# ExaScience/elprep

Measured on AMD Instinct MI355X. Metric: Mreads/s through sort+markdup+BQSR, 150bp PE, higher is better.
Workload: dtype u8/int32/int64 (integer path; float64 finalize on host)

## Files before the change

elprep_amd/csrc/bqsr.hip:

```cpp
#include <utility>

#include "bqsr_common.hpp"

namespace elp {

__global__ __launch_bounds__(256) void k_pack_reference(const uint8_t *__restrict__ ascii, int64_t len, uint8_t *__restrict__ packed, int64_t packed_bytes) {
  const int64_t i = (int64_t)blockIdx.x * blockDim.x + threadIdx.x;
  if (i >= packed_bytes) return;
  uint32_t out = 0;
  for (int h = 0; h < 2; h++) {
    const int64_t j = 2 * i + h;
    uint32_t code = 8;
    if (j < len) {
      switch (ascii[j]) {
        case 'a': case 'A': case '*': code = 0; break;
        case 'c': case 'C': code = 1; break;
        case 'g': case 'G': code = 2; break;
        case 't': case 'T': code = 3; break;
        default: code = 8;
      }
    }
    out |= code << (4 * h);
  }
  packed[i] = (uint8_t)out;
// ... 175 lines not shown
  ELP_TRY(fetch_err(c, e));
  if (e[0]) return bqsr_error(c, e[0]);
  const int64_t *hp = static_cast<const int64_t *>(c->h_pinned);
  memcpy(qual_tbl, hp, nq * 8);
  memcpy(cycle_tbl, hp + nq, nc * 8);
  memcpy(ctx_tbl, hp + nq + nc, nx * 8);
  return 0;
}

static int gather_impl(elp_ctx *c, int max_cycle, int64_t *qual_tbl, int64_t *cycle_tbl, int64_t *ctx_tbl) {
  for (int r = 0; r < c->n_ref; r++)
    if (!c->h_ref_seq[r]) return set_error(c, ELP_ERR_ARG, "elp_bqsr_gather: no reference sequence set for refid %d", r);
  for (int r = 0; r < c->n_ref; r++)
    if (!c->h_sites[r]) ELP_TRY(elp_bqsr_set_known_sites(c, r, nullptr, 0));
  ELP_TRY(sync_bqsr_ptrs(c));
  ELP_TRY(ensure_adapted(c, false));
  ELP_TRY(ensure_flat_index(c));
  ELP_TRY(ensure_qual_present(c));
  if (c->n_cov > 255) return set_error(c, ELP_ERR_UNSUPPORTED, "more than 255 read-group covariates");
  if (c->cigar_ops + 4 * c->n >= 0x7FFFFFFFull) return set_error(c, ELP_ERR_UNSUPPORTED, "CIGAR pool exceeds 2^31 operations per context");
  const int ncyc_g = 2 * max_cycle + 1;
  const size_t nq = (size_t)c->n_cov * ELP_NQUAL * 2, nc = nq * ncyc_g, nx = nq * ELP_NCTX;
  c->tables_n = 0;
  ELP_TRY(ensure(c, c->dev_tables, nq + nc + nx + elp_ctx::TABLES_TAIL));
  unsigned long long *tb = c->dev_tables.p;
  hipStream_t st = c->stream;
  ELP_HIP(c, hipMemsetAsync(tb, 0, (nq + nc + nx) * sizeof(unsigned long long), st));
  const uint64_t n = c->n;
  if (n && c->qual_bytes) {
    const GatherScratch S(n);
    PrologueBufs b;
    ELP_TRY(scratch(c, 1, 2 * (c->cigar_ops + 4 * n) + 64, &b.cs_pool));
    ELP_TRY(scratch(c, 2, n + 4, &b.desc));
    ELP_TRY(scratch(c, 0, 4 * n + 8, &b.plain_rec));
    const size_t skip_words = (size_t)((c->qual_bytes + 31) / 32 + 8);
    ELP_TRY(scratch(c, 3, skip_words, &b.skipbits));
    ELP_TRY(ensure_uniform_len(c));
    ELP_TRY(scratch(c, 5, S.words, &b.block));
    ELP_HIP(c, hipMemsetAsync(b.block, 0, 16, st));
    const GatherShape g{c->n_cov, (int)std::max<uint32_t>(c->max_l_seq, 1), max_cycle, c->uniform_len, c->tune.count_kernel, c->tune.count3_rlog,
                        COUNT3_STATIC_LDS, COUNT_STATIC_LDS, COUNT_STATIC_LDS_1024};
    uint32_t ncs = 1;
    while ((int)ncs < c->n_cov) ncs <<= 1;
    int mode = c3_mode(g, (int)quality_slots(c).size());
    if (S.too_many()) return set_error(c, ELP_ERR_UNSUPPORTED, "BQSR: more than ~1.4 G records per context");
    RecOut ro;
    ELP_TRY(rec_buffers(c, S, b.block, mode, ncs, &ro));
    if (!ro.recs) ELP_HIP(c, hipMemsetAsync(b.skipbits, 0, skip_words * 4, st));
    ELP_TRY(prologue_launch(c, b, S, ro));
    if (g.lmax > MAX_DESC_READ) return set_error(c, ELP_ERR_UNSUPPORTED, "BQSR: read longer than %d bases", MAX_DESC_READ);
    for (int attempt = 0;; attempt++) {
      const std::vector<int> quals = quality_slots(c);
      const CountPlan p = count_general_plan(g, (int)quals.size());
      if (!p.fits) return set_error(c, ELP_ERR_UNSUPPORTED, "BQSR: one covariate's private table rows do not fit in LDS (max read length=%d)", g.lmax);
      const int mode2 = ro.recs ? c3_mode(g, (int)quals.size()) : mode;
      if (mode2 != mode) {
        mode = mode2;
        ELP_TRY(rec_buffers(c, S, b.block, mode, ncs, &ro));
        ELP_HIP(c, hipMemsetAsync(b.skipbits, 0, skip_words * 4, st));
        ELP_HIP(c, hipMemsetAsync(b.block, 0, 16, st));
        ELP_TRY(prologue_launch(c, b, S, ro));
      }
      if (ro.recs) ELP_TRY(count_one_length(c, g, S, b, ro, quals, tb + nq, tb + nq + nc));
      else ELP_TRY(count_general(c, g, p, b, quals, tb + nq, tb + nq + nc));
      uint32_t e[4];
      ELP_TRY(fetch_err(c, e));
      if ((e[0] & ~128u) != 0) return bqsr_error(c, e[0] & ~128u);
// ... 160 lines not shown
```

elprep_amd/csrc/bqsr_common.hpp:

```cpp
#pragma once
#include "bqsr_dev.hpp"
#include "bqsr_plan.hpp"
#include "flat.hpp"

namespace elp {

constexpr int MAX_DESC_READ = 65535;


constexpr int32_t BQ_NOREF = INT32_MIN;
enum : uint8_t { BQ_ELIGIBLE = 1, BQ_REVERSED = 2, BQ_LAST = 4, BQ_CIG_SCRATCH = 8, BQ_COMPLEX = 16 };
struct __attribute__((aligned(16))) BqDesc {
  int32_t D0, D1, D2;
  int32_t refid;
  uint16_t b1, b2;
  uint16_t a;
  uint16_t len;
  uint16_t left;
  uint16_t right;
  uint8_t cov;
  uint8_t fl;
  uint16_t pad;
};
static_assert(sizeof(BqDesc) == 32, "BqDesc is staged as two 16-byte words");
// ... 231 lines not shown
  int rsw, rlog;
  unsigned long long *cycle_tbl, *ctx_tbl;
  uint32_t *err;
};
int count3_launch(elp_ctx *c, const Count3Args &A, const QMap &qm, size_t dyn);

struct CountArgs {
  uint64_t n, qual_bytes;
  const uint64_t *qual_off, *seq_off;
  const uint8_t *qual, *seq4;
  const BqDesc *desc;
  const uint32_t *cigar, *cig_scratch;
  const uint8_t *skipbits;
  uint8_t *const *ref_seq;
  const int64_t *ref_seq_len;
  int n_ref, n_cov, n_q, lmax, rs, max_cycle;
  unsigned long long *cycle_tbl, *ctx_tbl;
  uint32_t *err;
  const uint32_t *tile_first;
  int cov0;
};

int count_general_launch(elp_ctx *c, const CountArgs &A, const QMap &qm, const CountPlan &p, size_t dyn);
int qual_from_cycle_launch(elp_ctx *c, int ncyc_g, const unsigned long long *cycle_tbl, unsigned long long *qual_tbl);
int c3_segments_launch(elp_ctx *c, const GatherScratch &S, uint32_t *block, uint32_t nseg, uint32_t ncs);
int c3_other_sort_launch(elp_ctx *c, const uint4 *other, const uint32_t *n_other, uint32_t *cw, uint4 *sorted);

struct PrologueBufs {
  BqDesc *desc;
  uint32_t *skipbits;
  uint32_t *block;
  uint32_t *cs_pool;
  uint4 *plain_rec;
};
int prologue_launch(elp_ctx *c, const PrologueBufs &b, const GatherScratch &S, const RecOut &ro);

extern const size_t COUNT3_STATIC_LDS;
extern const size_t COUNT_STATIC_LDS, COUNT_STATIC_LDS_1024;
extern const size_t APPLY3_STATIC_LDS;

int bqsr_error(elp_ctx *c, uint32_t e);

int apply3_launch(elp_ctx *c, int max_cycle, const uint8_t *d_lut, const uint8_t *d_cov_present, const uint16_t *t1, const uint8_t *t2, const uint32_t *n_dict_dev,
                  int n_qi, int lmax, size_t dyn, bool split );

}
```

elprep_amd/csrc/bqsr_plan.hpp:

```cpp
#pragma once
#include <algorithm>
#include <cstddef>
#include <cstdint>

namespace elp {

constexpr size_t LDS_CU = 160 * 1024;

constexpr int CT_CYC = 32, CT_XROWS = 3, CT_PAD = 64;
constexpr int C3_XROWS = 3, C3_PAD = 64;
constexpr int C3_NSEG = 64;
constexpr int C3_MAXSEG = 256;
constexpr int C3_CSTRIDE = 64;
constexpr int PF_TILES = 16;
constexpr int CO_MAXCOV = 256;
constexpr int A3_ROW = 20;

inline int count3_plan(int n_cov, int n_q, int lmax, size_t static_lds, int *rsw_out, int *rlog_out, size_t *dyn_out, int force_rlog = -1) {
  const int ncw = ((17 * 2 * lmax) >> 4) + 2;
  const size_t rows = (size_t)n_cov * (size_t)(n_q + C3_XROWS);
  for (int rlog = 5; rlog >= 1; rlog--) {
    if (force_rlog >= 0 && force_rlog != rlog) continue;
    const int rsw = ((16 << rlog) + 16 + ncw + 31) & ~31;
    const size_t dyn = (rows * (size_t)rsw + C3_PAD) * 4;
    if (dyn + static_lds <= LDS_CU && rows * (size_t)rsw * 4 < (1u << 22)) {
      *rsw_out = rsw; *rlog_out = rlog; *dyn_out = dyn;
      return 0;
    }
  }
  return 1;
}

inline int apply3_bytes(int n_cov, int n_qi, int lmax, size_t static_lds, size_t *dyn_out) {
  const size_t n1 = (size_t)n_cov * (size_t)(6 + n_qi + 1) * (size_t)(2 * lmax + 1);
  const size_t dyn = ((n1 + 15) & ~(size_t)15) + (size_t)256 * A3_ROW + 16;
  *dyn_out = dyn;
  return dyn + static_lds <= LDS_CU ? 0 : 1;
}

struct GatherShape {
  int n_cov, lmax, max_cycle;
  uint32_t uniform_len;
  int count_kernel, count3_rlog;
  size_t lds_count3, lds_count, lds_count1024;
};

inline int c3_mode(const GatherShape &g, int nq) {
// ... 43 lines not shown
  p.passes = split(p.rs, &p.ncp, &p.qcap);
  if (p.passes != 1) {
    const int rs_mg = count_row_words(g.lmax, true);
    int ncp_mg = 0, qcap_mg = 0;
    const long passes_mg = split(rs_mg, &ncp_mg, &qcap_mg);
    if (passes_mg && (!p.passes || passes_mg < p.passes)) { p.mg = true; p.rs = rs_mg; p.ncp = ncp_mg; p.qcap = qcap_mg; p.passes = passes_mg; }
  }
  p.fits = p.qcap >= 1;
  return p;
}

struct GatherScratch {
  uint64_t n;
  size_t queue, plist, rec_cnt, cw, seg_cap, seg_base;
  size_t words;
  unsigned pf_grid;
  uint64_t cap_s1;
  explicit GatherScratch(uint64_t n_records) : n(n_records) {
    queue = 4;
    plist = (size_t)n + 20;
    rec_cnt = (size_t)((2 * n + 48 + 63) & ~(uint64_t)63);
    cw = rec_cnt + (size_t)(C3_MAXSEG + 1) * C3_CSTRIDE;
    seg_cap = cw + 3 * CO_MAXCOV + 1;
    seg_base = seg_cap + C3_MAXSEG;
    words = 2 * (size_t)n + 128 + (size_t)(C3_MAXSEG + 1) * C3_CSTRIDE + 4 * CO_MAXCOV + 2 * C3_MAXSEG + 32;
    pf_grid = (unsigned)((n + 256 * PF_TILES - 1) / (256 * PF_TILES));
    cap_s1 = ((uint64_t)pf_grid * 4 + C3_NSEG - 1) / C3_NSEG * (uint64_t)(PF_TILES * 64);
  }
  uint64_t other_at(int mode) const { return mode == 2 ? n : (uint64_t)C3_NSEG * cap_s1; }
  size_t rec_slots(int mode) const { return (size_t)other_at(mode) + (mode == 2 ? 2 : 1) * (size_t)n + 64; }
  bool too_many() const { return (uint64_t)C3_NSEG * cap_s1 + 2 * n >= 0xFFFFFFF0ull; }
};

}
```

elprep_amd/csrc/bqsr_prologue.hip:

```cpp
#include "bqsr_common.hpp"

namespace elp {

struct BqCols {
  uint64_t n;
  const int32_t *refid, *pos, *next_refid, *pnext, *tlen;
  const uint16_t *flag, *rgid;
  const uint8_t *mapq, *has_sr;
  const uint32_t *l_seq;
  const uint64_t *cigar_off, *seq_off, *qual_off;
  const uint32_t *cigar;
  const uint8_t *seq4;
  const uint8_t *qual;
  const int32_t *ref_len;
  const uint16_t *rg_cov;
  int32_t n_ref;
  uint8_t *const *ref_seq;
  const int64_t *ref_seq_len;
  int32_t *const *sites;
  const int64_t *n_sites;
  uint32_t *const *site_idx;
  const uint64_t *qbounds;
};

__device__ inline bool recalibrate_aln(const BqCols &m, uint64_t i) {
  if (m.has_sr[i]) return false;
  const uint8_t mq = m.mapq[i];
  if (!(mq > 0 && mq < 255)) return false;
  const uint16_t f = m.flag[i];
  if (f & (F_SECONDARY | F_DUPLICATE | F_QCFAILED)) return false;
  const int32_t r = m.refid[i], p = m.pos[i];
  if ((f & F_UNMAPPED) || r < 0 || p == 0) return false;
  if (!(p > 0)) return false;
  const uint32_t ls = m.l_seq[i];
  if (ls == 0) return false;
  if ((uint64_t)ls != m.qual_off[i + 1] - m.qual_off[i]) return false;
  if (m.rgid[i] == ELP_NIL16) return false;
  if (!(r < m.n_ref && p <= m.ref_len[r])) return false;
  int32_t rl = 0, refl = 0;
  for (uint64_t k = m.cigar_off[i]; k < m.cigar_off[i + 1]; k++) {
    const uint32_t c = m.cigar[k];
    if (c_op(c) == OP_N) return false;
    if (op_consumes_read(c_op(c))) rl += c_len(c);
    if (op_consumes_ref(c_op(c))) refl += c_len(c);
  }
  return refl >= 0 && (int32_t)ls == rl;
}

__device__ inline bool build_pieces(const uint32_t *cig, int ncig, int32_t pos, BqDesc &d) {
  int64_t val[3];
  bool noref[3];
  int start[3];
  int np = 0;
  int c = 0;
  int64_t delta = (int64_t)pos - 1;
// ... 23 lines not shown
    if (val[k] <= (int64_t)INT32_MIN + 70000 || val[k] >= (int64_t)INT32_MAX - 70000) return false;
    D[k] = (int32_t)val[k];
  }
  d.D0 = D[0]; d.D1 = D[1]; d.D2 = D[2];
  d.b1 = np > 1 ? (uint16_t)start[1] : (uint16_t)0xFFFF;
  d.b2 = np > 2 ? (uint16_t)start[2] : (uint16_t)0xFFFF;
  return true;
}

__device__ __forceinline__ void set_skip_bits(uint32_t *skipbits, uint64_t bit0, int fs, int fe) {
  for (int k = fs; k <= fe;) {
    const uint64_t b = bit0 + (uint64_t)k;
    const int in_word = (int)(b & 31);
    int cnt = 32 - in_word;
    if (cnt > fe - k + 1) cnt = fe - k + 1;
    const uint32_t mask = (cnt == 32 ? 0xFFFFFFFFu : ((1u << cnt) - 1u)) << in_word;
    atomicOr(&skipbits[b >> 5], mask);
    k += cnt;
  }
}

__device__ __forceinline__ void clear_skip_bits(uint32_t *skipbits, uint64_t bit0, uint32_t nbits) {
  for (uint32_t k = 0; k < nbits;) {
    const uint64_t b = bit0 + (uint64_t)k;
    const uint32_t in_word = (uint32_t)(b & 31);
    uint32_t cnt = 32 - in_word;
    if (cnt > nbits - k) cnt = nbits - k;
    const uint32_t mask = (cnt == 32 ? 0xFFFFFFFFu : ((1u << cnt) - 1u)) << in_word;
    atomicAnd(&skipbits[b >> 5], ~mask);
    k += cnt;
  }
}

struct PfCols {
  uint8_t has_sr, mq;
  uint16_t f, rg;
  int32_t r, p, pnext, tlen, nrefid;
  uint32_t ls;
  uint64_t q0, q1, c0, c1, qb;
};
__device__ __forceinline__ PfCols pf_load_cols(const BqCols &m, uint64_t i) {
  PfCols c;
  c.has_sr = m.has_sr[i]; c.mq = m.mapq[i]; c.f = m.flag[i]; c.rg = m.rgid[i];
  c.r = m.refid[i]; c.p = m.pos[i]; c.pnext = m.pnext[i]; c.tlen = m.tlen[i]; c.nrefid = m.next_refid[i];
  c.ls = m.l_seq[i];
  c.q0 = m.qual_off[i]; c.q1 = m.qual_off[i + 1]; c.c0 = m.cigar_off[i]; c.c1 = m.cigar_off[i + 1];
  c.qb = m.qbounds[i];
  return c;
}
struct PfLds {
  int32_t ref_len[REF_LDS];
  const int32_t *sites[REF_LDS];
  int64_t nsites[REF_LDS];
  const uint32_t *sidx[REF_LDS];
};
__device__ __forceinline__ void pf_lds_fill(PfLds &L, const BqCols &m, int nt) {
  if (m.n_ref <= REF_LDS)
    for (int r = threadIdx.x; r < m.n_ref; r += nt) { L.ref_len[r] = m.ref_len[r]; L.sites[r] = m.sites[r]; L.nsites[r] = m.n_sites[r]; L.sidx[r] = m.site_idx[r]; }
}

template <bool PLAIN_PASS>
__device__ __forceinline__ void pf_record(const BqCols &m, const uint64_t i, const PfCols &cur, const PfLds &L, const bool ref_lds, BqDesc *__restrict__ desc,
                                          uint32_t *skipbits, uint32_t *err, const bool recs , uint32_t *my_cig_w, bool &defer, bool &to_plain,
                                          BqRec &rc_out, int &rc_class, uint4 *__restrict__ plain_rec ,
                                          const uint32_t *pre_ops ) {
    const uint8_t has_sr = cur.has_sr, mq = cur.mq;
    const uint16_t f = cur.f, rg = cur.rg;
    const int32_t r = cur.r, p = cur.p, pnext = cur.pnext, tlen = cur.tlen, nrefid = cur.nrefid;
    const uint32_t ls = cur.ls;
    const uint64_t q0 = cur.q0, q1 = cur.q1, c0 = cur.c0, c1 = cur.c1;
    const uint64_t qb = cur.qb;
    BqDesc d;
    d.D0 = d.D1 = d.D2 = BQ_NOREF; d.refid = 0; d.b1 = d.b2 = 0xFFFF; d.a = 0; d.len = 0; d.left = 0; d.right = 0; d.cov = 0; d.fl = 0; d.pad = 0;
    const uint8_t *rec_rp = nullptr;
    int64_t rec_rlen = 0;
    bool used_col = false, rec_skipped_walk = false;
    bool ok = !has_sr && mq > 0 && mq < 255 && !(f & (F_SECONDARY | F_DUPLICATE | F_QCFAILED)) && !(f & F_UNMAPPED) && r >= 0 && p > 0 && ls != 0 &&
              (uint64_t)ls == q1 - q0 && rg != ELP_NIL16 && r < m.n_ref;
    if (ok) {
      const uint64_t nop = c1 - c0;
      if (recs) { rec_rp = m.ref_seq[r]; rec_rlen = m.ref_seq_len[r]; }
      uint32_t opv[5];
#pragma unroll
      for (int k = 0; k < 5; k++) opv[k] = PLAIN_PASS ? pre_ops[k] : ((uint64_t)k < nop ? m.cigar[c0 + k] : 0u);
      const int32_t rl = ref_lds ? L.ref_len[r] : m.ref_len[r];
      const uint16_t cov_rg = m.rg_cov[rg];
      const int32_t *sv = ref_lds ? L.sites[r] : m.sites[r];
      const int64_t ns = ref_lds ? L.nsites[r] : m.n_sites[r];
      auto bucket_entry = [&]() __attribute__((always_inline)) -> int64_t {
        const int64_t nbuck = ((int64_t)rl >> 6) + 1;
        int64_t bk = (int64_t)(p < rl ? p : rl) >> 6;
        bk = bk >= nbuck ? nbuck - 1 : bk;
        return (int64_t)(ref_lds ? L.sidx[r] : m.site_idx[r])[bk];
      };
      int64_t s_first = 0;
      if (!recs && ns > 0) s_first = bucket_entry();
      ok = p <= rl;
      bool simple = nop >= 1 && nop <= 5;
      uint32_t aoff = 0, mlen = 0, trail = 0;
      {
        uint32_t k = 0;
        if (simple && c_op(opv[0]) == OP_H) k = 1;
        auto at = [&](uint32_t j) { return j == 0 ? opv[0] : (j == 1 ? opv[1] : (j == 2 ? opv[2] : (j == 3 ? opv[3] : opv[4]))); };
        if (simple && k < nop && c_op(at(k)) == OP_S) { aoff = (uint32_t)c_len(at(k)); k++; }
        if (simple && k < nop && (c_op(at(k)) == OP_M || c_op(at(k)) == OP_EQ || c_op(at(k)) == OP_X)) { mlen = (uint32_t)c_len(at(k)); k++; }
        else simple = false;
        if (simple && k < nop && c_op(at(k)) == OP_S) { trail = (uint32_t)c_len(at(k)); k++; }
        if (simple && k < nop && c_op(at(k)) == OP_H) k++;
        simple = simple && k == nop && mlen != 0;
      }
      bool plain = false;
      uint32_t plain_read = 0, plain_ref = 0;
      if (!simple && nop >= 2 && nop <= 5) {
        plain = true;
#pragma unroll
        for (int k = 0; k < 5; k++) {
          if ((uint64_t)k < nop) {
            const uint32_t o = c_op(opv[k]), ln = (uint32_t)c_len(opv[k]);
            if (o == OP_M || o == OP_EQ || o == OP_X) { plain_read += ln; plain_ref += ln; }
            else if (o == OP_I) plain_read += ln;
            else if (o == OP_D) plain_ref += ln;
            else plain = false;
          }
        }
      }
      if (!PLAIN_PASS) {
        if (ok && plain && ls <= (uint32_t)MAX_DESC_READ) {
          uint4 *pr = plain_rec + 4 * i;
          pr[0] = make_uint4(opv[0], opv[1], opv[2], opv[3]);
          pr[1] = make_uint4(opv[4], (uint32_t)f | ((uint32_t)rg << 16), (uint32_t)r, (uint32_t)p);
          pr[2] = make_uint4(ls | ((uint32_t)nop << 16) | (nrefid < 0 ? 1u << 19 : 0u), (uint32_t)c0, (uint32_t)q0, (uint32_t)(q0 >> 32));
          pr[3] = make_uint4((uint32_t)qb, (uint32_t)(qb >> 32), (uint32_t)pnext, (uint32_t)tlen);
          to_plain = true;
          return;
        }
        plain = false;
      } else if (plain) {
#pragma unroll
        for (int k = 0; k < 5; k++) my_cig_w[k] = opv[k];
      }
      const uint32_t *my_cig = my_cig_w;
      if (ok && !((simple || plain) && ls <= (uint32_t)MAX_DESC_READ)) { defer = true; ok = false; }
      if (ok) ok = (plain ? plain_read : aoff + mlen + trail) == ls;
      if (ok) {
        const int len = plain ? (int)ls : (int)mlen;
        const int32_t end = p + (plain ? (int)plain_ref : len) - 1;
        const bool rev = f & F_REVERSED;
        bool clip = false;
        if (tlen != 0 && (f & F_MULTIPLE) && !((f & F_NEXT_UNMAPPED) || nrefid < 0 || pnext == 0) && rev != (bool)(f & F_NEXT_REVERSED)) {
          const bool well = rev ? end > pnext : p <= pnext + tlen;
          if (well) {
            const int boundary = rev ? (int)pnext - 1 : (int)p + (tlen < 0 ? -(int)tlen : (int)tlen);
            clip = boundary >= (int)p && boundary <= (int)end;
          }
        }
        const uint32_t hi1 = (uint32_t)qb;
        int left = len, right = len - 1;
        if (!clip && hi1) {
          const int f0 = (int)(qb >> 32) - (int)aoff, l0 = (int)hi1 - 1 - (int)aoff;
          if (f0 < len && l0 >= 0) {
            if (f0 >= 0) left = f0;
            else if (m.qual[q0 + aoff] > 2) left = 0;
            else clip = true;
            if (l0 < len) right = l0;
            else if (m.qual[q0 + aoff + (uint32_t)len - 1] > 2) right = len - 1;
            else clip = true;
// ... 45 lines not shown
            d.b1 = (uint16_t)nop;
            d.D2 = p - 1;
          }
          d.left = (uint16_t)left; d.right = (uint16_t)(right < 0 ? 0xFFFF : right);
          d.cov = (uint8_t)cov_rg;
          d.fl = BQ_ELIGIBLE | (rev ? BQ_REVERSED : 0) | ((f & F_LAST) ? BQ_LAST : 0) | complex_fl;
        }
      }
    }
    if (!defer) {
      if (recs) {
        BqRec rc;
        rc.ref_lo = rc.ref_hi = rc.win = rc.ctxw = 0; rc.t0 = 0; rc.fl = rc.bpk = rc.dpk = 0;
        if (d.fl & BQ_ELIGIBLE) {
          Pieces4 P;
          if (d.fl & BQ_COMPLEX) pieces4(my_cig_w, (int)(c1 - c0), p, P);
          else if (d.b1 != 0xFFFFu) pieces4(my_cig_w, (int)(c1 - c0), p, P);
          else { P.v0 = (int64_t)d.D0; P.v1 = P.v2 = P.v3 = 0; P.s1 = P.s2 = P.s3 = 0; P.noref = d.D0 == BQ_NOREF ? 1u : 0u; P.np = 1; }
          rc = make_rec((int)d.a, (int)d.len, (int)d.left, d.right == 0xFFFFu ? -1 : (int)d.right, d.cov, (d.fl & BQ_REVERSED) != 0, (d.fl & BQ_LAST) != 0, P,
                        P.np < 0, rec_rp, rec_rlen, (int64_t)ls);
          if (used_col) rc.fl |= RC_SKIPCOL;
          else if ((rc.fl & RC_GENERAL) && rec_skipped_walk) atomicOr(&err[0], 1024u);
        }
        if (rc.fl & RC_GENERAL) desc[i] = d;
        rc_class = rec_class(rc);
        rec_pack_idx(rc, (uint32_t)i);
        rc_out = rc;
      } else {
        desc[i] = d;
      }
    }
}

__global__ __launch_bounds__(256) void k_bqsr_prologue_fast(BqCols m, BqDesc *__restrict__ desc, uint32_t *skipbits, uint32_t *__restrict__ queue,
                                                            uint32_t *queue_n, uint32_t *err, RecOut ro, uint32_t *__restrict__ plist, uint4 *__restrict__ plain_rec) {
  __shared__ uint32_t lq[PF_TILES * 256];
  __shared__ uint32_t lcount, gbase, pcount, pbase;
  __shared__ uint32_t seg_n[C3_MAXSEG], seg_at[C3_MAXSEG];
  __shared__ PfLds L;
  const bool ref_lds = m.n_ref <= REF_LDS;
  pf_lds_fill(L, m, 256);
  if (threadIdx.x == 0) { lcount = 0; pcount = 0; }
  seg_n[threadIdx.x] = 0;
  __syncthreads();
  const uint64_t i_first = (uint64_t)blockIdx.x * PF_TILES * 256 + threadIdx.x;
  PfCols nxt = {};
  if (i_first < m.n) nxt = pf_load_cols(m, i_first);
#pragma unroll 1
  for (int tile = 0; tile < PF_TILES; tile++) {
    const uint64_t i = i_first + (uint64_t)tile * 256;
    bool defer = false, to_plain = false;
    const PfCols cur = nxt;
    if (tile + 1 < PF_TILES && i + 256 < m.n) nxt = pf_load_cols(m, i + 256);
    BqRec rc;
    int rcl = 0;
    if (i < m.n) pf_record<false>(m, i, cur, L, ref_lds, desc, skipbits, err, ro.recs != nullptr, nullptr, defer, to_plain, rc, rcl, plain_rec, nullptr);
    if (ro.recs) {
      if (!ro.ncs) {
        const uint32_t seg = (blockIdx.x * 4u + (threadIdx.x >> 6)) % ro.nseg;
        const uint32_t at1 = wave_append(rcl == 1, &ro.cnt[seg * C3_CSTRIDE]);
        if (rcl == 1) rec_store(ro.recs, (uint64_t)ro.seg_base[seg] + at1, rc);
      } else {
        const uint32_t cov = rc.fl & 0xFFu, seg = (blockIdx.x % (ro.nseg / ro.ncs)) * ro.ncs + cov;
        uint32_t rank = 0;
        if (rcl == 1) rank = atomicAdd(&seg_n[cov], 1u);
        __syncthreads();
        if (threadIdx.x < ro.ncs) {
          const uint32_t t = seg_n[threadIdx.x];
          if (t) {
            seg_at[threadIdx.x] = atomicAdd(&ro.cnt[((blockIdx.x % (ro.nseg / ro.ncs)) * ro.ncs + threadIdx.x) * C3_CSTRIDE], t);
            seg_n[threadIdx.x] = 0;
          }
        }
        __syncthreads();
        if (rcl == 1) rec_store(ro.recs, (uint64_t)ro.seg_base[seg] + seg_at[cov] + rank, rc);
      }
      const uint32_t at2 = wave_append(rcl == 2, &ro.cnt[ro.nseg * C3_CSTRIDE]);
      if (rcl == 2) rec_store(ro.recs, ro.other_at + at2, rc);
    }
    const int lane = threadIdx.x & 63;
    const unsigned long long mask = __ballot(defer);
    if (mask) {
      const int leader = __ffsll((long long)mask) - 1;
      uint32_t base = 0;
      if (lane == leader) base = atomicAdd(&lcount, (uint32_t)__popcll(mask));
      base = __shfl(base, leader, 64);
      if (defer) lq[base + (uint32_t)__popcll(mask & ((1ull << lane) - 1ull))] = (uint32_t)i;
    }
    const unsigned long long pmask = __ballot(to_plain);
    if (pmask) {
      const int leader = __ffsll((long long)pmask) - 1;
      uint32_t base = 0;
      if (lane == leader) base = atomicAdd(&pcount, (uint32_t)__popcll(pmask));
      base = __shfl(base, leader, 64);
      if (to_plain) lq[PF_TILES * 256 - 1 - (base + (uint32_t)__popcll(pmask & ((1ull << lane) - 1ull)))] = (uint32_t)i;
    }
  }
  __syncthreads();
  if (threadIdx.x == 0) {
    gbase = lcount ? atomicAdd(queue_n, lcount) : 0u;
    pbase = pcount ? atomicAdd(queue_n + 1, pcount) : 0u;
  }
  __syncthreads();
  for (uint32_t k = threadIdx.x; k < lcount; k += 256) queue[gbase + k] = lq[k];
  for (uint32_t k = threadIdx.x; k < pcount; k += 256) plist[pbase + k] = lq[PF_TILES * 256 - 1 - k];
}

__global__ __launch_bounds__(256) void k_bqsr_prologue_plain(BqCols m, BqDesc *__restrict__ desc, uint32_t *skipbits, const uint32_t *__restrict__ plist,
                                                             uint32_t *__restrict__ queue, uint32_t *queue_n, uint32_t *err, RecOut ro, const uint4 *__restrict__ plain_rec) {
  __shared__ uint32_t s_cig[256][5];
  __shared__ uint32_t wg_n, wg_base, wr_n, wr_base;
  __shared__ PfLds L;
  const bool ref_lds = m.n_ref <= REF_LDS;
  pf_lds_fill(L, m, 256);
  __syncthreads();
  const uint64_t np = (uint64_t)queue_n[1];
  const uint64_t stride = (uint64_t)gridDim.x * 256;
  for (uint64_t t0 = (uint64_t)blockIdx.x * 256; t0 < np; t0 += stride) {
    const uint64_t t = t0 + threadIdx.x;
    bool defer = false, to_plain = false;
    uint32_t i = 0;
    BqRec rc;
    int rcl = 0;
    if (t < np) {
      i = plist[t];
      const uint4 *pr = plain_rec + 4 * (size_t)i;
      const uint4 w0 = pr[0], w1 = pr[1], w2 = pr[2], w3 = pr[3];
      const uint32_t ops[5] = {w0.x, w0.y, w0.z, w0.w, w1.x};
      PfCols cur;
      cur.has_sr = 0; cur.mq = 1;
      cur.f = (uint16_t)w1.y; cur.rg = (uint16_t)(w1.y >> 16);
      cur.r = (int32_t)w1.z; cur.p = (int32_t)w1.w;
      cur.ls = w2.x & 0xFFFFu;
      cur.nrefid = (w2.x >> 19) & 1u ? -1 : 0;
      cur.c0 = (uint64_t)w2.y; cur.c1 = cur.c0 + ((w2.x >> 16) & 7u);
      cur.q0 = (uint64_t)w2.z | ((uint64_t)w2.w << 32); cur.q1 = cur.q0 + cur.ls;
      cur.qb = (uint64_t)w3.x | ((uint64_t)w3.y << 32);
      cur.pnext = (int32_t)w3.z; cur.tlen = (int32_t)w3.w;
      pf_record<true>(m, i, cur, L, ref_lds, desc, skipbits, err, ro.recs != nullptr, s_cig[threadIdx.x], defer, to_plain, rc, rcl, nullptr, ops);
    }
    if (threadIdx.x == 0) { wg_n = 0; wr_n = 0; }
    __syncthreads();
    uint32_t my = 0, myr = 0;
    if (defer) my = atomicAdd(&wg_n, 1u);
    if (rcl) myr = atomicAdd(&wr_n, 1u);
    __syncthreads();
    if (threadIdx.x == 0) {
      wg_base = wg_n ? atomicAdd(queue_n, wg_n) : 0u;
      wr_base = wr_n ? atomicAdd(&ro.cnt[ro.nseg * C3_CSTRIDE], wr_n) : 0u;
    }
    __syncthreads();
    if (defer) queue[wg_base + my] = i;
    if (rcl) rec_store(ro.recs, ro.other_at + wr_base + myr, rc);
  }
}

__device__ inline void prologue_general(const BqCols &m, const uint64_t i, uint32_t *__restrict__ cig_scratch, BqDesc *__restrict__ desc, uint32_t *skipbits,
                                        uint32_t *err, const bool recs, BqRec &rc_out, int &rc_class) {
  int32_t rec_pos = 0;
  auto put = [&](const BqDesc &dd, const uint32_t *cg, int ncg) {
    if (!recs) { desc[i] = dd; return; }
    BqRec rc;
    rc.ref_lo = rc.ref_hi = rc.win = rc.ctxw = 0; rc.t0 = 0; rc.fl = rc.bpk = rc.dpk = 0;
    if (dd.fl & BQ_ELIGIBLE) {
      Pieces4 P;
      pieces4(cg, ncg, rec_pos, P);
      rc = make_rec((int)dd.a, (int)dd.len, (int)dd.left, dd.right == 0xFFFFu ? -1 : (int)dd.right, dd.cov, (dd.fl & BQ_REVERSED) != 0, (dd.fl & BQ_LAST) != 0, P,
                    P.np < 0, m.ref_seq[dd.refid], m.ref_seq_len[dd.refid], (int64_t)m.l_seq[i]);
      rc.fl |= RC_SKIPCOL;
    }
    if (rc.fl & RC_GENERAL) desc[i] = dd;
    rc_class = rec_class(rc) ? 2 : 0;
// ... 59 lines not shown
    d.D2 = a.pos - 1;
    if (a.ncig > 0xFFFF) atomicOr(&err[0], 2u);
  }
  put(d, a.cig, a.ncig);
}

__global__ __launch_bounds__(256) void k_bqsr_prologue(BqCols m, const uint32_t *__restrict__ queue, const uint32_t *__restrict__ queue_n,
                                                       uint32_t *__restrict__ cig_scratch, BqDesc *__restrict__ desc, uint32_t *skipbits,
                                                       uint32_t *err, RecOut ro) {
  __shared__ uint32_t wr_n, wr_base;
  const uint64_t nq = (uint64_t)*queue_n;
  const uint64_t stride = (uint64_t)gridDim.x * blockDim.x;
  for (uint64_t t0 = (uint64_t)blockIdx.x * blockDim.x; t0 < nq; t0 += stride) {
    const uint64_t t = t0 + threadIdx.x;
    BqRec rc;
    int rcl = 0;
    if (t < nq) prologue_general(m, queue[t], cig_scratch, desc, skipbits, err, ro.recs != nullptr, rc, rcl);
    if (!ro.recs) continue;
    if (threadIdx.x == 0) wr_n = 0;
    __syncthreads();
    uint32_t myr = 0;
    if (rcl) myr = atomicAdd(&wr_n, 1u);
    __syncthreads();
    if (threadIdx.x == 0) wr_base = wr_n ? atomicAdd(&ro.cnt[ro.nseg * C3_CSTRIDE], wr_n) : 0u;
    __syncthreads();
    if (rcl) rec_store(ro.recs, ro.other_at + wr_base + myr, rc);
  }
}

int prologue_launch(elp_ctx *c, const PrologueBufs &b, const GatherScratch &S, const RecOut &ro) {
  const uint64_t n = c->n;
  BqCols m{n, c->refid.p, c->pos.p, c->next_refid.p, c->pnext.p, c->tlen.p, c->flag.p, c->rgid.p, c->mapq.p, c->has_sr.p, c->l_seq.p,
           c->cigar_off.p, c->seq_off.p, c->qual_off.p, c->cigar.p, c->seq4.p, c->qual.p, c->ref_len.p, c->rg_cov.p, c->n_ref,
           c->d_ref_seq.p, c->d_ref_seq_len.p, c->d_sites.p, c->d_n_sites.p, c->d_site_idx.p, c->qbounds.p};
  uint32_t *queue_n = b.block, *queue = b.block + S.queue, *plist = b.block + S.plist;
  ELP_LAUNCH(c, "bqsr_prologue_fast", k_bqsr_prologue_fast, dim3(S.pf_grid), dim3(256), 0, m, b.desc, b.skipbits, queue, queue_n, c->err_flag.p, ro, plist, b.plain_rec);
  const unsigned grid = std::min<unsigned>(blocks_for(n, 256), (unsigned)c->n_cu * 16);
  ELP_LAUNCH(c, "bqsr_prologue_plain", k_bqsr_prologue_plain, dim3(grid), dim3(256), 0, m, b.desc, b.skipbits, (const uint32_t *)plist, queue, queue_n, c->err_flag.p, ro,
             (const uint4 *)b.plain_rec);
  ELP_LAUNCH(c, "bqsr_prologue", k_bqsr_prologue, dim3(grid), dim3(256), 0, m, (const uint32_t *)queue, (const uint32_t *)queue_n, b.cs_pool, b.desc, b.skipbits,
             c->err_flag.p, ro);
  return 0;
}

}
```

elprep_amd/csrc/common.hpp:

```cpp
#pragma once

#include <hip/hip_runtime.h>

#include <sched.h>

#include <cstdarg>
#include <cstdint>
#include <cstdio>
#include <cstring>
#include <map>
#include <mutex>
#include <string>
#include <vector>

#include "../../include/elprep_hip.h"
#include "../../include/elprep_hip_debug.h"
#include "derived.hpp"

namespace elp {

constexpr int WAVE = 64;

enum : uint16_t {
  F_MULTIPLE = 0x1, F_PROPER = 0x2, F_UNMAPPED = 0x4, F_NEXT_UNMAPPED = 0x8, F_REVERSED = 0x10, F_NEXT_REVERSED = 0x20,
// ... 165 lines not shown
  bool sort_ahead = false;
  uint64_t presort_n = 0;
  uint64_t *presort_ks = nullptr;
  int presort_idx_bits = 0;

  elp::DVec<uint16_t> snap_flag;
  elp::DVec<uint8_t> snap_qual;
  uint64_t snap_n = 0, snap_qual_bytes = 0;

  struct Tuning {
    int count_kernel = 0;
    int apply_kernel = 0;
    int count3_rlog = -1;
    int qual_hint = 0;
    int qual_hint_drop = -1;
    int pair_table_slots = 1 << 20;
    long long bgzf_piece = 1ll << 30;
    int bgzf_weak_guess = 0;
    int score_kernel = 0;
    int mate_path = 0;
    int radix_tile = 0;
    int sort_pairs = 0;
    int tie_rounds = 0;
    int exchange_piece = 0;
    int emit_pass = 0;
    long long bgzf_inflate_piece = 2ll << 30;
    int bgzf_copy_chunk = 0;
    int bgzf_tok_lds = 0;
    int bgzf_first_chunk_div = 4;
    int bgzf_fixed = 0;
    int bgzf_tok_fail_above = 0;
    int bgzf_stored = 0;
    int apply_wgs = 0;
    int count3_grid = 0;
    int presort_tile = 0;
    int side_priority = 0;
  } tune;

  elp::DVec<uint8_t> scratch[8];

  bool profiling = false;
  const char *prof_prefix = nullptr;
  std::vector<std::string> prof_names;
  std::map<std::string, int> prof_index;
  std::vector<uint64_t> prof_launches;
  std::vector<double> prof_ms;
  std::vector<elp::ProfPending> prof_pending;
};

namespace elp {

int set_error(elp_ctx *c, int code, const char *fmt, ...);
int prof_begin(elp_ctx *c, const char *name);
void prof_end(elp_ctx *c, int pending);
int prof_flush(elp_ctx *c);
struct ProfScope {
  elp_ctx *c;
  const char *saved;
  ProfScope(elp_ctx *ctx, const char *prefix) : c(ctx), saved(ctx->prof_prefix) { ctx->prof_prefix = prefix; }
  ~ProfScope() { c->prof_prefix = saved; }
};

#define ELP_HIP(ctx, call)                                                                             \
  do {                                                                                                 \
    hipError_t e__ = (call);                                                                           \
    if (e__ != hipSuccess)                                                                             \
// ... 186 lines not shown
```

elprep_amd/csrc/ctx.hip:

```cpp
#include "common.hpp"

namespace elp {

namespace {
constexpr size_t GUARD = 4096;
constexpr uint8_t GUARD_BYTE = 0xC3;
std::mutex guard_mu;
std::map<void *, size_t> guard_of;
int guard_check_one(void *p, size_t payload) {
  uint8_t host[GUARD];
  if (hipDeviceSynchronize() != hipSuccess || hipMemcpy(host, static_cast<uint8_t *>(p) + payload, GUARD, hipMemcpyDeviceToHost) != hipSuccess) return 0;
  for (size_t k = 0; k < GUARD; k++)
    if (host[k] != GUARD_BYTE) {
      fprintf(stderr, "[elp] ELP_DEBUG_GUARD: byte %zu behind the end of a %zu-byte device buffer was overwritten (0x%02x)\n", k, payload, host[k]);
      return 1;
    }
  return 0;
}
}
size_t debug_guard_bytes() {
  static const size_t v = [] { const char *e = getenv("ELP_DEBUG_GUARD"); return (e && *e && *e != '0') ? GUARD : (size_t)0; }();
  return v;
}
void debug_guard_arm(void *p, size_t payload) {
// ... 564 lines not shown
  if (k == "count_kernel") c->tune.count_kernel = v;
  else if (k == "apply_kernel") c->tune.apply_kernel = v;
  else if (k == "bgzf_piece") { if (value < 1) return set_error(c, ELP_ERR_ARG, "elp_set_tuning: bgzf_piece must be positive"); c->tune.bgzf_piece = value; }
  else if (k == "bgzf_weak_guess") c->tune.bgzf_weak_guess = v;
  else if (k == "score_kernel") { c->tune.score_kernel = v; c->derived.score_tuning_changed(); }
  else if (k == "count3_rlog") c->tune.count3_rlog = v;
  else if (k == "qual_hint") { c->tune.qual_hint = v; c->derived.hint_tuning_changed(); }
  else if (k == "qual_hint_drop") { c->tune.qual_hint_drop = v; c->derived.hint_tuning_changed(); }
  else if (k == "pair_table_slots") {
    if (v == 0) { c->tune.pair_table_slots = 1 << 20; return 0; }
    if (v < 2 || v > (1 << 20) || (v & (v - 1))) return set_error(c, ELP_ERR_ARG, "elp_set_tuning: pair_table_slots must be a power of two >= 2");
    c->tune.pair_table_slots = v;
  } else if (k == "mate_path") {
    if (value != 0 && value != 2) return set_error(c, ELP_ERR_ARG, "elp_set_tuning: mate_path is 0 (the library decides) or 2 (every candidate through the table)");
    c->tune.mate_path = v;
  } else if (k == "tie_rounds") c->tune.tie_rounds = v;
  else if (k == "radix_tile") c->tune.radix_tile = v;
  else if (k == "sort_pairs") c->tune.sort_pairs = v;
  else if (k == "exchange_piece") c->tune.exchange_piece = v;
  else if (k == "emit_pass") c->tune.emit_pass = v;
  else if (k == "bgzf_stored") c->tune.bgzf_stored = v;
  else if (k == "bgzf_tok_fail_above") c->tune.bgzf_tok_fail_above = v;
  else if (k == "bgzf_fixed") c->tune.bgzf_fixed = v;
  else if (k == "bgzf_first_chunk_div") c->tune.bgzf_first_chunk_div = v;
  else if (k == "bgzf_tok_lds") c->tune.bgzf_tok_lds = v;
  else if (k == "bgzf_copy_chunk") c->tune.bgzf_copy_chunk = v;
  else if (k == "bgzf_inflate_piece") { if (value < 1) return set_error(c, ELP_ERR_ARG, "elp_set_tuning: bgzf_inflate_piece must be positive"); c->tune.bgzf_inflate_piece = value; }
  else if (k == "md_fused" || k == "bgzf_inflate") {
    if (value != 0) return set_error(c, ELP_ERR_ARG, "elp_set_tuning: key '%s' is retired (only 0 is accepted)", key);
  } else if (k == "apply_wgs") c->tune.apply_wgs = v;
  else if (k == "presort_tile") c->tune.presort_tile = v;
  else if (k == "count3_grid") { if (value < 0) return set_error(c, ELP_ERR_ARG, "elp_set_tuning: count3_grid must not be negative"); c->tune.count3_grid = v; }
  else if (k == "side_priority") c->tune.side_priority = v;
  else return set_error(c, ELP_ERR_ARG, "elp_set_tuning: unknown key '%s'", key);
  return 0;
}

int elp_profile_enable(elp_ctx *c, int on) {
  if (!c) return ELP_ERR_ARG;
  if (!on) { ELP_TRY(prof_flush(c)); prof_merge_side(c); }
  c->profiling = on != 0;
  for (int lane = 0; lane < 2; lane++)
    if (c->side[lane]) c->side[lane]->profiling = c->profiling;
  return 0;
}
int elp_profile_reset(elp_ctx *c) {
  if (!c) return ELP_ERR_ARG;
  ELP_TRY(prof_flush(c));
  prof_merge_side(c);
  for (auto &v : c->prof_launches) v = 0;
  for (auto &v : c->prof_ms) v = 0.0;
  return 0;
}
int elp_profile_count(elp_ctx *c) {
  if (!c) return ELP_ERR_ARG;
  if (prof_flush(c) != 0) return ELP_ERR_HIP;
  prof_merge_side(c);
  return (int)c->prof_names.size();
}
int elp_profile_get(elp_ctx *c, int index, const char **name, uint64_t *launches, double *total_ms) {
  if (!c || index < 0 || index >= (int)c->prof_names.size()) return ELP_ERR_ARG;
  if (name) *name = c->prof_names[index].c_str();
  if (launches) *launches = c->prof_launches[index];
  if (total_ms) *total_ms = c->prof_ms[index];
  return 0;
}
// ... 3 lines not shown
```

Measured before the change: 2407.

## Compact BQSR prologue hand-over records per workgroup and skip per-read offsets for uniform lengths

The fast prologue kernel now writes plain-record hand-over lines into a per-workgroup compacted buffer capped at a tunable size, instead of a 64-byte slot per read indexed by read id. The plain pass finds each line through a per-workgroup base offset, and falls back to reloading the columns from global memory when a line was past the cap. For uniform read lengths, a templated variant derives the quality offsets from the index and skips loading l_seq and qual_off. The reference sequence pointers and read-group covariate map are also staged in LDS. The aim is less scratch memory and less global traffic, at the cost of more code paths and an extra fallback path when overflow occurs.

```diff
diff --git a/elprep_amd/csrc/bqsr.hip b/elprep_amd/csrc/bqsr.hip
--- a/elprep_amd/csrc/bqsr.hip
+++ b/elprep_amd/csrc/bqsr.hip
@@ -231,7 +231,8 @@
     PrologueBufs b;
     ELP_TRY(scratch(c, 1, 2 * (c->cigar_ops + 4 * n) + 64, &b.cs_pool));
     ELP_TRY(scratch(c, 2, n + 4, &b.desc));
-    ELP_TRY(scratch(c, 0, 4 * n + 8, &b.plain_rec));
+    b.pl = plain_rec_plan(S, c->tune.prologue_plain_cap);
+    ELP_TRY(scratch(c, 0, b.pl.units, &b.plain_rec));
     const size_t skip_words = (size_t)((c->qual_bytes + 31) / 32 + 8);
     ELP_TRY(scratch(c, 3, skip_words, &b.skipbits));
     ELP_TRY(ensure_uniform_len(c));
diff --git a/elprep_amd/csrc/bqsr_common.hpp b/elprep_amd/csrc/bqsr_common.hpp
--- a/elprep_amd/csrc/bqsr_common.hpp
+++ b/elprep_amd/csrc/bqsr_common.hpp
@@ -287,6 +287,7 @@
   uint32_t *block;
   uint32_t *cs_pool;
   uint4 *plain_rec;
+  PlainRecPlan pl;
 };
 int prologue_launch(elp_ctx *c, const PrologueBufs &b, const GatherScratch &S, const RecOut &ro);
 
diff --git a/elprep_amd/csrc/bqsr_plan.hpp b/elprep_amd/csrc/bqsr_plan.hpp
--- a/elprep_amd/csrc/bqsr_plan.hpp
+++ b/elprep_amd/csrc/bqsr_plan.hpp
@@ -13,6 +13,8 @@
 constexpr int C3_MAXSEG = 256;
 constexpr int C3_CSTRIDE = 64;
 constexpr int PF_TILES = 16;
+constexpr uint32_t PL_CAP = 1024;
+constexpr int RG_LDS = 256;
 constexpr int CO_MAXCOV = 256;
 constexpr int A3_ROW = 20;
 
@@ -122,4 +124,18 @@
   bool too_many() const { return (uint64_t)C3_NSEG * cap_s1 + 2 * n >= 0xFFFFFFF0ull; }
 };
 
+struct PlainRecPlan {
+  uint32_t cap;
+  size_t wg_base_at;
+  size_t units;
+  size_t bytes() const { return units * 16; }
+};
+inline PlainRecPlan plain_rec_plan(const GatherScratch &S, int tune_cap) {
+  PlainRecPlan p;
+  p.cap = std::min<uint32_t>(tune_cap > 0 ? (uint32_t)tune_cap : PL_CAP, (uint32_t)PF_TILES * 256);
+  p.wg_base_at = 4 * (size_t)S.pf_grid * p.cap;
+  p.units = p.wg_base_at + ((size_t)S.pf_grid + 3) / 4 + 2;
+  return p;
 }
+
+}
diff --git a/elprep_amd/csrc/bqsr_prologue.hip b/elprep_amd/csrc/bqsr_prologue.hip
--- a/elprep_amd/csrc/bqsr_prologue.hip
+++ b/elprep_amd/csrc/bqsr_prologue.hip
@@ -1,3 +1,5 @@
+#include <type_traits>
+
 #include "bqsr_common.hpp"
 
 namespace elp {
@@ -21,6 +23,8 @@
   const int64_t *n_sites;
   uint32_t *const *site_idx;
   const uint64_t *qbounds;
+  uint32_t uniform_len;
+  int32_t n_rg;
 };
 
 __device__ inline bool recalibrate_aln(const BqCols &m, uint64_t i) {
@@ -110,19 +114,23 @@
   }
 }
 
-struct PfCols {
+struct PfColsU {
   uint8_t has_sr, mq;
   uint16_t f, rg;
   int32_t r, p, pnext, tlen, nrefid;
+  uint64_t c0, c1, qb;
+};
+struct PfCols : PfColsU {
   uint32_t ls;
-  uint64_t q0, q1, c0, c1, qb;
+  uint64_t q0, q1;
 };
-__device__ __forceinline__ PfCols pf_load_cols(const BqCols &m, uint64_t i) {
-  PfCols c;
+template <class COLS>
+__device__ __forceinline__ COLS pf_load_cols(const BqCols &m, uint64_t i) {
+  COLS c;
   c.has_sr = m.has_sr[i]; c.mq = m.mapq[i]; c.f = m.flag[i]; c.rg = m.rgid[i];
   c.r = m.refid[i]; c.p = m.pos[i]; c.pnext = m.pnext[i]; c.tlen = m.tlen[i]; c.nrefid = m.next_refid[i];
-  c.ls = m.l_seq[i];
-  c.q0 = m.qual_off[i]; c.q1 = m.qual_off[i + 1]; c.c0 = m.cigar_off[i]; c.c1 = m.cigar_off[i + 1];
+  if constexpr (std::is_same<COLS, PfCols>::value) { c.ls = m.l_seq[i]; c.q0 = m.qual_off[i]; c.q1 = m.qual_off[i + 1]; }
+  c.c0 = m.cigar_off[i]; c.c1 = m.cigar_off[i + 1];
   c.qb = m.qbounds[i];
   return c;
 }
@@ -131,23 +139,42 @@
   const int32_t *sites[REF_LDS];
   int64_t nsites[REF_LDS];
   const uint32_t *sidx[REF_LDS];
+  const uint8_t *ref_seq[REF_LDS];
+  int64_t ref_seq_len[REF_LDS];
+  uint16_t rg_cov[RG_LDS];
 };
 __device__ __forceinline__ void pf_lds_fill(PfLds &L, const BqCols &m, int nt) {
   if (m.n_ref <= REF_LDS)
-    for (int r = threadIdx.x; r < m.n_ref; r += nt) { L.ref_len[r] = m.ref_len[r]; L.sites[r] = m.sites[r]; L.nsites[r] = m.n_sites[r]; L.sidx[r] = m.site_idx[r]; }
-}
-
-template <bool PLAIN_PASS>
-__device__ __forceinline__ void pf_record(const BqCols &m, const uint64_t i, const PfCols &cur, const PfLds &L, const bool ref_lds, BqDesc *__restrict__ desc,
-                                          uint32_t *skipbits, uint32_t *err, const bool recs , uint32_t *my_cig_w, bool &defer, bool &to_plain,
-                                          BqRec &rc_out, int &rc_class, uint4 *__restrict__ plain_rec ,
+    for (int r = threadIdx.x; r < m.n_ref; r += nt) {
+      L.ref_len[r] = m.ref_len[r]; L.sites[r] = m.sites[r]; L.nsites[r] = m.n_sites[r]; L.sidx[r] = m.site_idx[r];
+      L.ref_seq[r] = m.ref_seq[r]; L.ref_seq_len[r] = m.ref_seq_len[r];
+    }
+  if (m.n_rg <= RG_LDS)
+    for (int g = threadIdx.x; g < m.n_rg; g += nt) L.rg_cov[g] = m.rg_cov[g];
+}
+struct PfList {
+  uint32_t *lq, *pcount;
+  uint4 *lines;
+  uint32_t cap;
+};
+
+template <bool PLAIN_PASS, bool UNI>
+__device__ __forceinline__ void pf_record(const BqCols &m, const uint64_t i, const typename std::conditional<UNI, PfColsU, PfCols>::type &cur, const PfLds &L,
+                                          const bool ref_lds, BqDesc *__restrict__ desc, uint32_t *skipbits, uint32_t *err, const bool recs ,
+                                          uint32_t *my_cig_w, bool &defer, BqRec &rc_out, int &rc_class,
+                                          const PfList &pl ,
                                           const uint32_t *pre_ops ) {
+    static_assert(!(PLAIN_PASS && UNI), "the second pass takes the offsets from the hand-over line");
     const uint8_t has_sr = cur.has_sr, mq = cur.mq;
     const uint16_t f = cur.f, rg = cur.rg;
     const int32_t r = cur.r, p = cur.p, pnext = cur.pnext, tlen = cur.tlen, nrefid = cur.nrefid;
-    const uint32_t ls = cur.ls;
-    const uint64_t q0 = cur.q0, q1 = cur.q1, c0 = cur.c0, c1 = cur.c1;
+    uint32_t ls;
+    uint64_t q0, q1;
+    if constexpr (UNI) { ls = m.uniform_len; q0 = i * (uint64_t)ls; q1 = q0 + ls; }
+    else { ls = cur.ls; q0 = cur.q0; q1 = cur.q1; }
+    const uint64_t c0 = cur.c0, c1 = cur.c1;
     const uint64_t qb = cur.qb;
+    const bool rg_lds = m.n_rg <= RG_LDS;
     BqDesc d;
     d.D0 = d.D1 = d.D2 = BQ_NOREF; d.refid = 0; d.b1 = d.b2 = 0xFFFF; d.a = 0; d.len = 0; d.left = 0; d.right = 0; d.cov = 0; d.fl = 0; d.pad = 0;
     const uint8_t *rec_rp = nullptr;
@@ -157,12 +184,12 @@
               (uint64_t)ls == q1 - q0 && rg != ELP_NIL16 && r < m.n_ref;
     if (ok) {
       const uint64_t nop = c1 - c0;
-      if (recs) { rec_rp = m.ref_seq[r]; rec_rlen = m.ref_seq_len[r]; }
+      if (recs) { rec_rp = ref_lds ? L.ref_seq[r] : m.ref_seq[r]; rec_rlen = ref_lds ? L.ref_seq_len[r] : m.ref_seq_len[r]; }
       uint32_t opv[5];
 #pragma unroll
       for (int k = 0; k < 5; k++) opv[k] = PLAIN_PASS ? pre_ops[k] : ((uint64_t)k < nop ? m.cigar[c0 + k] : 0u);
       const int32_t rl = ref_lds ? L.ref_len[r] : m.ref_len[r];
-      const uint16_t cov_rg = m.rg_cov[rg];
+      const uint16_t cov_rg = rg_lds ? L.rg_cov[rg] : m.rg_cov[rg];
       const int32_t *sv = ref_lds ? L.sites[r] : m.sites[r];
       const int64_t ns = ref_lds ? L.nsites[r] : m.n_sites[r];
       auto bucket_entry = [&]() __attribute__((always_inline)) -> int64_t {
@@ -204,12 +231,19 @@
       }
       if (!PLAIN_PASS) {
         if (ok && plain && ls <= (uint32_t)MAX_DESC_READ) {
-          uint4 *pr = plain_rec + 4 * i;
-          pr[0] = make_uint4(opv[0], opv[1], opv[2], opv[3]);
-          pr[1] = make_uint4(opv[4], (uint32_t)f | ((uint32_t)rg << 16), (uint32_t)r, (uint32_t)p);
-          pr[2] = make_uint4(ls | ((uint32_t)nop << 16) | (nrefid < 0 ? 1u << 19 : 0u), (uint32_t)c0, (uint32_t)q0, (uint32_t)(q0 >> 32));
-          pr[3] = make_uint4((uint32_t)qb, (uint32_t)(qb >> 32), (uint32_t)pnext, (uint32_t)tlen);
-          to_plain = true;
+          const unsigned long long pm = __ballot(true);
+          const int lane = threadIdx.x & 63;
+          uint32_t base = 0;
+          if (lane == __ffsll((long long)pm) - 1) base = atomicAdd(pl.pcount, (uint32_t)__popcll(pm));
+          const uint32_t rank = (uint32_t)__builtin_amdgcn_readfirstlane((int)base) + (uint32_t)__popcll(pm & ((1ull << lane) - 1ull));
+          pl.lq[PF_TILES * 256 - 1 - rank] = (uint32_t)i;
+          if (rank < pl.cap) {
+            uint4 *pr = pl.lines + 4 * (size_t)rank;
+            pr[0] = make_uint4(opv[0], opv[1], opv[2], opv[3]);
+            pr[1] = make_uint4(opv[4], (uint32_t)f | ((uint32_t)rg << 16), (uint32_t)r, (uint32_t)p);
+            pr[2] = make_uint4(ls | ((uint32_t)nop << 16) | (nrefid < 0 ? 1u << 19 : 0u), (uint32_t)c0, (uint32_t)q0, (uint32_t)(q0 >> 32));
+            pr[3] = make_uint4((uint32_t)qb, (uint32_t)(qb >> 32), (uint32_t)pnext, (uint32_t)tlen);
+          }
           return;
         }
         plain = false;
@@ -321,8 +355,11 @@
     }
 }
 
+template <bool UNI>
 __global__ __launch_bounds__(256) void k_bqsr_prologue_fast(BqCols m, BqDesc *__restrict__ desc, uint32_t *skipbits, uint32_t *__restrict__ queue,
-                                                            uint32_t *queue_n, uint32_t *err, RecOut ro, uint32_t *__restrict__ plist, uint4 *__restrict__ plain_rec) {
+                                                            uint32_t *queue_n, uint32_t *err, RecOut ro, uint32_t *__restrict__ plist, uint4 *__restrict__ plain_rec,
+                                                            uint32_t plain_cap, uint32_t *__restrict__ plain_wg_base) {
+  using Cols = typename std::conditional<UNI, PfColsU, PfCols>::type;
   __shared__ uint32_t lq[PF_TILES * 256];
   __shared__ uint32_t lcount, gbase, pcount, pbase;
   __shared__ uint32_t seg_n[C3_MAXSEG], seg_at[C3_MAXSEG];
@@ -333,17 +370,18 @@
   seg_n[threadIdx.x] = 0;
   __syncthreads();
   const uint64_t i_first = (uint64_t)blockIdx.x * PF_TILES * 256 + threadIdx.x;
-  PfCols nxt = {};
-  if (i_first < m.n) nxt = pf_load_cols(m, i_first);
+  const PfList pl{lq, &pcount, plain_rec + 4 * (size_t)blockIdx.x * plain_cap, plain_cap};
+  Cols nxt = {};
+  if (i_first < m.n) nxt = pf_load_cols<Cols>(m, i_first);
 #pragma unroll 1
   for (int tile = 0; tile < PF_TILES; tile++) {
     const uint64_t i = i_first + (uint64_t)tile * 256;
-    bool defer = false, to_plain = false;
-    const PfCols cur = nxt;
-    if (tile + 1 < PF_TILES && i + 256 < m.n) nxt = pf_load_cols(m, i + 256);
+    bool defer = false;
+    const Cols cur = nxt;
+    if (tile + 1 < PF_TILES && i + 256 < m.n) nxt = pf_load_cols<Cols>(m, i + 256);
     BqRec rc;
     int rcl = 0;
-    if (i < m.n) pf_record<false>(m, i, cur, L, ref_lds, desc, skipbits, err, ro.recs != nullptr, nullptr, defer, to_plain, rc, rcl, plain_rec, nullptr);
+    if (i < m.n) pf_record<false, UNI>(m, i, cur, L, ref_lds, desc, skipbits, err, ro.recs != nullptr, nullptr, defer, rc, rcl, pl, nullptr);
     if (ro.recs) {
       if (!ro.ncs) {
         const uint32_t seg = (blockIdx.x * 4u + (threadIdx.x >> 6)) % ro.nseg;
@@ -376,19 +414,12 @@
       base = __shfl(base, leader, 64);
       if (defer) lq[base + (uint32_t)__popcll(mask & ((1ull << lane) - 1ull))] = (uint32_t)i;
     }
-    const unsigned long long pmask = __ballot(to_plain);
-    if (pmask) {
-      const int leader = __ffsll((long long)pmask) - 1;
-      uint32_t base = 0;
-      if (lane == leader) base = atomicAdd(&pcount, (uint32_t)__popcll(pmask));
-      base = __shfl(base, leader, 64);
-      if (to_plain) lq[PF_TILES * 256 - 1 - (base + (uint32_t)__popcll(pmask & ((1ull << lane) - 1ull)))] = (uint32_t)i;
-    }
   }
   __syncthreads();
   if (threadIdx.x == 0) {
     gbase = lcount ? atomicAdd(queue_n, lcount) : 0u;
     pbase = pcount ? atomicAdd(queue_n + 1, pcount) : 0u;
+    plain_wg_base[blockIdx.x] = pbase;
   }
   __syncthreads();
   for (uint32_t k = threadIdx.x; k < lcount; k += 256) queue[gbase + k] = lq[k];
@@ -396,7 +427,8 @@
 }
 
 __global__ __launch_bounds__(256) void k_bqsr_prologue_plain(BqCols m, BqDesc *__restrict__ desc, uint32_t *skipbits, const uint32_t *__restrict__ plist,
-                                                             uint32_t *__restrict__ queue, uint32_t *queue_n, uint32_t *err, RecOut ro, const uint4 *__restrict__ plain_rec) {
+                                                             uint32_t *__restrict__ queue, uint32_t *queue_n, uint32_t *err, RecOut ro, const uint4 *__restrict__ plain_rec,
+                                                             uint32_t plain_cap, const uint32_t *__restrict__ plain_wg_base) {
   __shared__ uint32_t s_cig[256][5];
   __shared__ uint32_t wg_n, wg_base, wr_n, wr_base;
   __shared__ PfLds L;
@@ -407,26 +439,34 @@
   const uint64_t stride = (uint64_t)gridDim.x * 256;
   for (uint64_t t0 = (uint64_t)blockIdx.x * 256; t0 < np; t0 += stride) {
     const uint64_t t = t0 + threadIdx.x;
-    bool defer = false, to_plain = false;
+    bool defer = false;
     uint32_t i = 0;
     BqRec rc;
     int rcl = 0;
     if (t < np) {
       i = plist[t];
-      const uint4 *pr = plain_rec + 4 * (size_t)i;
-      const uint4 w0 = pr[0], w1 = pr[1], w2 = pr[2], w3 = pr[3];
-      const uint32_t ops[5] = {w0.x, w0.y, w0.z, w0.w, w1.x};
+      const uint32_t wg = i / (uint32_t)(PF_TILES * 256), k = (uint32_t)t - plain_wg_base[wg];
       PfCols cur;
-      cur.has_sr = 0; cur.mq = 1;
-      cur.f = (uint16_t)w1.y; cur.rg = (uint16_t)(w1.y >> 16);
-      cur.r = (int32_t)w1.z; cur.p = (int32_t)w1.w;
-      cur.ls = w2.x & 0xFFFFu;
-      cur.nrefid = (w2.x >> 19) & 1u ? -1 : 0;
-      cur.c0 = (uint64_t)w2.y; cur.c1 = cur.c0 + ((w2.x >> 16) & 7u);
-      cur.q0 = (uint64_t)w2.z | ((uint64_t)w2.w << 32); cur.q1 = cur.q0 + cur.ls;
-      cur.qb = (uint64_t)w3.x | ((uint64_t)w3.y << 32);
-      cur.pnext = (int32_t)w3.z; cur.tlen = (int32_t)w3.w;
-      pf_record<true>(m, i, cur, L, ref_lds, desc, skipbits, err, ro.recs != nullptr, s_cig[threadIdx.x], defer, to_plain, rc, rcl, nullptr, ops);
+      uint32_t ops[5];
+      if (k < plain_cap) {
+        const uint4 *pr = plain_rec + 4 * ((size_t)wg * plain_cap + k);
+        const uint4 w0 = pr[0], w1 = pr[1], w2 = pr[2], w3 = pr[3];
+        ops[0] = w0.x; ops[1] = w0.y; ops[2] = w0.z; ops[3] = w0.w; ops[4] = w1.x;
+        cur.has_sr = 0; cur.mq = 1;
+        cur.f = (uint16_t)w1.y; cur.rg = (uint16_t)(w1.y >> 16);
+        cur.r = (int32_t)w1.z; cur.p = (int32_t)w1.w;
+        cur.ls = w2.x & 0xFFFFu;
+        cur.nrefid = (w2.x >> 19) & 1u ? -1 : 0;
+        cur.c0 = (uint64_t)w2.y; cur.c1 = cur.c0 + ((w2.x >> 16) & 7u);
+        cur.q0 = (uint64_t)w2.z | ((uint64_t)w2.w << 32); cur.q1 = cur.q0 + cur.ls;
+        cur.qb = (uint64_t)w3.x | ((uint64_t)w3.y << 32);
+        cur.pnext = (int32_t)w3.z; cur.tlen = (int32_t)w3.w;
+      } else {
+        cur = pf_load_cols<PfCols>(m, i);
+#pragma unroll
+        for (int j = 0; j < 5; j++) ops[j] = cur.c0 + (uint64_t)j < cur.c1 ? m.cigar[cur.c0 + j] : 0u;
+      }
+      pf_record<true, false>(m, i, cur, L, ref_lds, desc, skipbits, err, ro.recs != nullptr, s_cig[threadIdx.x], defer, rc, rcl, PfList{}, ops);
     }
     if (threadIdx.x == 0) { wg_n = 0; wr_n = 0; }
     __syncthreads();
@@ -552,12 +592,19 @@
   const uint64_t n = c->n;
   BqCols m{n, c->refid.p, c->pos.p, c->next_refid.p, c->pnext.p, c->tlen.p, c->flag.p, c->rgid.p, c->mapq.p, c->has_sr.p, c->l_seq.p,
            c->cigar_off.p, c->seq_off.p, c->qual_off.p, c->cigar.p, c->seq4.p, c->qual.p, c->ref_len.p, c->rg_cov.p, c->n_ref,
-           c->d_ref_seq.p, c->d_ref_seq_len.p, c->d_sites.p, c->d_n_sites.p, c->d_site_idx.p, c->qbounds.p};
+           c->d_ref_seq.p, c->d_ref_seq_len.p, c->d_sites.p, c->d_n_sites.p, c->d_site_idx.p, c->qbounds.p,
+           c->derived.has_uniform(c->n, c->qual_bytes) ? c->uniform_len : 0u, c->n_rg};
   uint32_t *queue_n = b.block, *queue = b.block + S.queue, *plist = b.block + S.plist;
-  ELP_LAUNCH(c, "bqsr_prologue_fast", k_bqsr_prologue_fast, dim3(S.pf_grid), dim3(256), 0, m, b.desc, b.skipbits, queue, queue_n, c->err_flag.p, ro, plist, b.plain_rec);
+  uint32_t *wg_base = reinterpret_cast<uint32_t *>(b.plain_rec + b.pl.wg_base_at);
+  if (ro.recs && m.uniform_len && m.uniform_len <= (uint32_t)MAX_DESC_READ && c->tune.prologue_uniform)
+    ELP_LAUNCH(c, "bqsr_prologue_fast", k_bqsr_prologue_fast<true>, dim3(S.pf_grid), dim3(256), 0, m, b.desc, b.skipbits, queue, queue_n, c->err_flag.p, ro, plist, b.plain_rec,
+               b.pl.cap, wg_base);
+  else
+    ELP_LAUNCH(c, "bqsr_prologue_fast", k_bqsr_prologue_fast<false>, dim3(S.pf_grid), dim3(256), 0, m, b.desc, b.skipbits, queue, queue_n, c->err_flag.p, ro, plist, b.plain_rec,
+               b.pl.cap, wg_base);
   const unsigned grid = std::min<unsigned>(blocks_for(n, 256), (unsigned)c->n_cu * 16);
   ELP_LAUNCH(c, "bqsr_prologue_plain", k_bqsr_prologue_plain, dim3(grid), dim3(256), 0, m, b.desc, b.skipbits, (const uint32_t *)plist, queue, queue_n, c->err_flag.p, ro,
-             (const uint4 *)b.plain_rec);
+             (const uint4 *)b.plain_rec, b.pl.cap, (const uint32_t *)wg_base);
   ELP_LAUNCH(c, "bqsr_prologue", k_bqsr_prologue, dim3(grid), dim3(256), 0, m, (const uint32_t *)queue, (const uint32_t *)queue_n, b.cs_pool, b.desc, b.skipbits,
              c->err_flag.p, ro);
   return 0;
diff --git a/elprep_amd/csrc/common.hpp b/elprep_amd/csrc/common.hpp
--- a/elprep_amd/csrc/common.hpp
+++ b/elprep_amd/csrc/common.hpp
@@ -221,6 +221,8 @@
     int bgzf_tok_fail_above = 0;
     int bgzf_stored = 0;
     int apply_wgs = 0;
+    int prologue_uniform = 1;
+    int prologue_plain_cap = 0;
     int count3_grid = 0;
     int presort_tile = 0;
     int side_priority = 0;
diff --git a/elprep_amd/csrc/ctx.hip b/elprep_amd/csrc/ctx.hip
--- a/elprep_amd/csrc/ctx.hip
+++ b/elprep_amd/csrc/ctx.hip
@@ -620,6 +620,8 @@
   else if (k == "presort_tile") c->tune.presort_tile = v;
   else if (k == "count3_grid") { if (value < 0) return set_error(c, ELP_ERR_ARG, "elp_set_tuning: count3_grid must not be negative"); c->tune.count3_grid = v; }
   else if (k == "side_priority") c->tune.side_priority = v;
+  else if (k == "prologue_uniform") c->tune.prologue_uniform = v;
+  else if (k == "prologue_plain_cap") { if (value < 0) return set_error(c, ELP_ERR_ARG, "elp_set_tuning: prologue_plain_cap must not be negative"); c->tune.prologue_plain_cap = v; }
   else return set_error(c, ELP_ERR_ARG, "elp_set_tuning: unknown key '%s'", key);
   return 0;
 }
```

After: 2394, median of 2. No clear change (-0.6%).
